# flysoaryun/LF-VIO

Hardware: AMD Instinct MI355X
Metric: sliding-window solves/sec (10 KF x N landmarks) (higher is better)
Workload: dtype f64; 1 GPU; window300; landmarks=300, observations=1419, windows_per_gpu=1, marginalization=MARGIN_OLD, parallelism=1 independent window stream(s), one per GPU, no data-path collective

## Files before the change

### lf-vio_amd/csrc/dev_types.h

```cpp
#pragma once
#include "../../include/lfvio.h"

constexpr int KC = 73;
constexpr int KP = 172;
constexpr int WLD = 80;
__host__ __device__ inline int w_row_len(int cnt) { return 6 * cnt + 9; }
constexpr int COL_B = 73;
constexpr int COL_K = 74;
constexpr int NQ = 105;
constexpr int NG = 210;
constexpr int NGP = 212;
constexpr int NPAIR = 121;
constexpr int NT = 15;
constexpr int SCHUR_LEN = NT * 256;
constexpr int PACKED = KP * (KP + 1) / 2;
constexpr int JMAX_SWEEPS = 20;
constexpr int PRE_CHUNK_LIMIT = 2 * 121;
constexpr int SUM_ITEMS_CAP = PRE_CHUNK_LIMIT * 209 + 64;
constexpr int SUM_VIS_PACKED = 73 * 74 / 2, SUM_VIS = SUM_VIS_PACKED + 73;
constexpr int HPP_CAP = 16384;
constexpr int XOFF_H = 0;
constexpr int XOFF_G = 14880;
constexpr int XOFF_S = XOFF_G + 176;
constexpr int XOFF_C = XOFF_S + 15 * 256;
// ... 167 lines not shown
  GP<int> lm_start, lm_cnt, lm_obs0, lm_perm;
  GP<int> lm_woff;
  GP<double> lam0;
  GP<double> obs[8];
  GP<int> pm_obs, pm_lm;
  GP<double> anc[8];
  GP<double> pmo[8];
  GP<unsigned char> pm_pair;
  GP<int> linb_lm0, linb_ns;
  GP<int> chunk_pair, chunk_begin, chunk_end;
  GP<double> prior_J, prior_r;
  GP<int> sum_off, sum_end_marg, sum_items;
  FrameState x[2];
  TRState tr;
  Tab tab[2];
  GP<double> lam[2];
  FrameState xE[SPEC_EXTRA];
  Tab tabE[SPEC_EXTRA];
  GP<double> lamE[SPEC_EXTRA];
  GP<double> cost_partE;
  double pose_costE[SPEC_EXTRA][16];
  double imu_sqrt[LFVIO_WINDOW_SIZE][225];
  GP<double> prior_A;
  double prior_b0[KP];
  GP<double> a, b, W, scale_l, grad_l, gn_l, diag_l, einv_l, d1, d2;
  GP<double> Wt;
  GP<double> gram_part, pairG, schur_part, schur_sum;
  GP<double> xch, gp;
  GP<double> lm_part;
  double lm_sum[LMS];
  GP<double> cost_part;
  GP<double> imu_out;
  GP<double> imu_raw;
  double prior_g[KP + 4];
  double pose_cost[16];
  GP<double> Hpp;
  GP<double> mscr;
  GP<double> eig_aux;
  double scale_p[KP], diag_p[KP], grad_p[KP], gn_p[KP], step_p[KP];
  double uc_grad[WLD], uc_gn[WLD];
  struct SpecCtl {
    int ep;
    int word;
    int fin;
    int ticket;
    int own[SPEC_OWN];
  } spec;
  struct SpecShadow {
    int hdr_ep;
    int word;
    int last_word;
    int ticket;
  } shadow;
  long long dbg[32];
  double jtrace[32];
  LfvioPrior prior_out;
};

struct PendingBlock {
  int open, passes;
  int tail_state, passes_used, iters_done, chain_err;
};
static_assert(offsetof(Slot, passes_used) - offsetof(Slot, tail_state) == offsetof(PendingBlock, passes_used) - offsetof(PendingBlock, tail_state) &&
                  offsetof(Slot, iters_done) - offsetof(Slot, tail_state) == offsetof(PendingBlock, iters_done) - offsetof(PendingBlock, tail_state) &&
                  offsetof(Slot, chain_err) - offsetof(Slot, tail_state) == offsetof(PendingBlock, chain_err) - offsetof(PendingBlock, tail_state),
              "PendingBlock mirrors Slot::tail_state .. chain_err");
```

### lf-vio_amd/csrc/kernels_marg.h

```cpp
#pragma once
#include "kernels_solve.h"

constexpr int MARG_THREADS = 768;
constexpr int MARG_MAXD = 96;
constexpr int LDN = 80;
constexpr double JACOBI_TOL = 1e-19;
constexpr size_t MARG_LDS = (size_t)19072 * sizeof(double);
constexpr int BT_GROUP = 4;

DEV void gauge_landmarks(Slot *S, int l0) {
  const int l = l0 + (int)threadIdx.x;
  double *lam = S->lam[S->tr.cur];
  if (l < S->N) lam[l] = 1.0 / (1.0 / lam[l]);
}
template <class T>
DEV void copy_rounds(T *dst, const T *src, int n, int tid, int nthr) {
  for (int k0 = tid; k0 < n; k0 += 8 * nthr) {
    T v[8];
#pragma unroll
    for (int q = 0; q < 8; q++) v[q] = src[k0 + q * nthr < n ? k0 + q * nthr : 0];
#pragma unroll
    for (int q = 0; q < 8; q++)
      if (k0 + q * nthr < n) dst[k0 + q * nthr] = v[q];
  }
// ... 561 lines not shown
#pragma unroll
  for (int i = P; i < 5; i++) {
    const double kv = K2 * vi[i];
#pragma unroll
    for (int q = P; q < 5; q++) ar[i][q] = fma(kv, vj[q], ar[i][q]);
    if (i == P) tri_finish_row<P>(tc, k + 1, ar[P], tc.r0 == ((k + 1) & 15));
  }
}
template <int QM, int NR>
DEV void bt_apply(const double *RV, const double *tau, int k, int n, int l8, double (&zz)[10]) {
  double vq[NR][10], tk[NR];
#pragma unroll
  for (int r = 0; r < NR; r++) {
    const int kr = k - r;
    const double *v = RV + kr * 76 - (kr + 1);
    tk[r] = tau[kr];
#pragma unroll
    for (int q = QM; q < 10; q++) {
      const int i = l8 + 8 * q;
      if (QM == 0) vq[r][q] = (i > kr && i < n) ? v[i] : 0.0;
      else vq[r][q] = (q > QM || i > kr) ? v[i] : 0.0;
    }
  }
#pragma unroll
  for (int r = 0; r < NR; r++) {
    double s0 = 0.0, s1 = 0.0;
#pragma unroll
    for (int q = QM; q < 10; q++) {
      if ((q - QM) & 1) s1 = fma(vq[r][q], zz[q], s1);
      else s0 = fma(vq[r][q], zz[q], s0);
    }
    const double s = sum8(s0 + s1) * tk[r];
#pragma unroll
    for (int q = QM; q < 10; q++) zz[q] = fma(-s, vq[r][q], zz[q]);
  }
}
template <int NR>
DEV void bt_dispatch(const double *RV, const double *tau, int k, int n, int l8, double (&zz)[10]) {
  switch (k >> 3) {
    case 0: bt_apply<0, NR>(RV, tau, k, n, l8, zz); break;
    case 1: bt_apply<1, NR>(RV, tau, k, n, l8, zz); break;
    case 2: bt_apply<2, NR>(RV, tau, k, n, l8, zz); break;
    case 3: bt_apply<3, NR>(RV, tau, k, n, l8, zz); break;
    case 4: bt_apply<4, NR>(RV, tau, k, n, l8, zz); break;
    case 5: bt_apply<5, NR>(RV, tau, k, n, l8, zz); break;
    case 6: bt_apply<6, NR>(RV, tau, k, n, l8, zz); break;
    case 7: bt_apply<7, NR>(RV, tau, k, n, l8, zz); break;
    case 8: bt_apply<8, NR>(RV, tau, k, n, l8, zz); break;
    default: bt_apply<9, NR>(RV, tau, k, n, l8, zz); break;
  }
}
DEV double guard_pivot(double q, double pivmin) { return copysign(fmax(fabs(q), pivmin), q); }
template <bool SPEC>
DEV bool eig_tridiag(double *A, const double *b, int n, int tid, double *RV, double *DM, double *vec, double *scr, double *nn2, double *Tglob, LfvioPrior *out, double eps, long long *dbg,
                     SpecPoll *sp_) {
  SpecPoll *const sp = SPEC ? sp_ : nullptr;
  const bool poller = SPEC && tid == MARG_THREADS - 1;
#define ESTAMP(k) do { if (tid == 0) dbg[k] = (long long)__builtin_readcyclecounter(); } while (0)
  ESTAMP(26);
  const int wave = tid >> 6, lane = tid & 63;
  double *dd = vec, *ee = vec + 96, *ee2 = vec + 192, *tau = vec + 288, *lam = vec + 384, *pp = vec + 480, *nrm = vec + 576;
  const bool tri = tid < 256;
  const int r0 = (tid >> 4) & 15, c0 = tid & 15;
  double ar[5][5];
#pragma unroll
  for (int i = 0; i < 5; i++)
#pragma unroll
    for (int q = 0; q < 5; q++) {
      const int R = r0 + 16 * i, C = c0 + 16 * q;
      ar[i][q] = (tri && R < n && C < n) ? A[max(R, C) * LDN + min(R, C)] : 0.0;
    }
  double *vb0 = lam, *vb1 = nrm;
  if (tid < 96) dd[tid] = 0.0, ee[tid] = 0.0, ee2[tid] = 0.0, tau[tid] = 0.0, vb0[tid] = 0.0, vb1[tid] = 0.0;
  for (int e = tid; e < 76 * 76; e += MARG_THREADS) RV[e] = 0.0;
  __syncthreads();
  TriCtx tc = {dd, ee, tau, vb0, vb1, pp, RV, n, r0, c0};
  if (tri) tri_finish_row<0>(tc, 0, ar[0], r0 == 0);
  __syncthreads();
  for (int k = 0; k + 2 < n; k++) {
    const int P = (k + 1) >> 4;
    double vj[5];
    if (poller) {
      if ((k & 7) == 0) spec_poll_issue(*sp);
      else if ((k & 7) == 6) spec_poll_take(*sp);
    }
#ifdef LFVIO_TRI_PROFILE
#define TSTAMP(j) do { if (tid == 0 && k == LFVIO_TRI_PROFILE) dbg[3 + j] = (long long)__builtin_readcyclecounter(); } while (0)
#else
#define TSTAMP(j) do { } while (0)
#endif
    TSTAMP(0);
    if (tri) {
      switch (P) {
        case 0: tri_matvec<0>(tc, k, ar, vj); break;
        case 1: tri_matvec<1>(tc, k, ar, vj); break;
        case 2: tri_matvec<2>(tc, k, ar, vj); break;
        case 3: tri_matvec<3>(tc, k, ar, vj); break;
        default: tri_matvec<4>(tc, k, ar, vj); break;
      }
    }
    TSTAMP(1);
    __syncthreads();
    TSTAMP(2);
    if (tri) {
      switch (P) {
        case 0: tri_update<0>(tc, k, ar, vj); break;
        case 1: tri_update<1>(tc, k, ar, vj); break;
        case 2: tri_update<2>(tc, k, ar, vj); break;
        case 3: tri_update<3>(tc, k, ar, vj); break;
        default: tri_update<4>(tc, k, ar, vj); break;
      }
    }
    TSTAMP(3);
    __syncthreads();
    TSTAMP(4);
    if (sp && (k & 7) == 6 && *sp->flag) return true;
  }
  if (tri) {
#pragma unroll
    for (int i = 0; i < 5; i++)
#pragma unroll
      for (int q = 0; q < 5; q++)
        if (r0 + 16 * i == n - 1 && c0 + 16 * q == n - 1) dd[n - 1] = ar[i][q];
  }
// ... 120 lines not shown
    __syncthreads();
    ESTAMP(17);
    if (sp && *sp->flag) return true;
    if (work) {
      const double g0 = pp[mec], g1 = pp[96 + mec];
      const int kt = g1 < g0 ? ((int *)ee2)[96 + mec] : ((int *)ee2)[mec];
      double z = 1.0, nn = 0.0;
      if (set == 0) {
        A[kt * LDN + mec] = 1.0;
        for (int i0 = n - 2; i0 >= 0; i0 -= 8) {
          double c[8], zs[8];
#pragma unroll
          for (int u = 0; u < 8; u++) {
            const int i = max(i0 - u, 0);
            c[u] = -ee[i] * fast_rcp(guard_pivot(A[i * LDN + mec], pivmin));
          }
#pragma unroll
          for (int u = 0; u < 8; u++) {
            const bool on = i0 - u < kt && i0 - u >= 0;
            z = on ? c[u] * z : 1.0;
            zs[u] = z;
            nn = on ? fma(z, z, nn) : nn;
          }
#pragma unroll
          for (int u = 0; u < 8; u++)
            if (i0 - u < kt && i0 - u >= 0) A[(i0 - u) * LDN + mec] = zs[u];
        }
      } else {
        for (int i0 = 1; i0 < n; i0 += 8) {
          double c[8], zs[8];
#pragma unroll
          for (int u = 0; u < 8; u++) {
            const int i = min(i0 + u, n - 1);
            c[u] = -ee[i - 1] * fast_rcp(guard_pivot(DM[i * LDN + mec], pivmin));
          }
#pragma unroll
          for (int u = 0; u < 8; u++) {
            const bool on = i0 + u > kt && i0 + u < n;
            z = on ? c[u] * z : 1.0;
            zs[u] = z;
            nn = on ? fma(z, z, nn) : nn;
          }
#pragma unroll
          for (int u = 0; u < 8; u++)
            if (i0 + u > kt && i0 + u < n) A[(i0 + u) * LDN + mec] = zs[u];
        }
      }
      nn2[set * 96 + mec] = nn;
    }
  }
  __syncthreads();
  ESTAMP(29);
  {
    const int m = tid >> 3, l8 = tid & 7;
    const bool live = m < n;
    const int mm = live ? m : 0;
    double zz[10];
    const double sc = fast_rsqrt(1.0 + nn2[mm] + nn2[96 + mm]);
#pragma unroll
    for (int q = 0; q < 10; q++) {
      const int i = l8 + 8 * q;
      zz[q] = i < n ? A[i * LDN + mm] * sc : 0.0;
    }
    int k = n - 3;
    for (; k >= 0 && (k & (BT_GROUP - 1)) != BT_GROUP - 1; k--) bt_dispatch<1>(RV, tau, k, n, l8, zz);
    for (; k >= 0; k -= BT_GROUP) bt_dispatch<BT_GROUP>(RV, tau, k, n, l8, zz);
    const double l = lam[mm];
    double rb = 0.0;
#pragma unroll
    for (int q = 0; q < 10; q++) {
      const int i = l8 + 8 * q;
      if (i < n) rb = fma(zz[q], b[i], rb);
    }
    rb = sum8(rb);
    if (live) {
      const bool keep = l > eps;
      const double sq = keep ? sqrt(l) : 0.0;
#pragma unroll
      for (int q = 0; q < 10; q++) {
        const int i = l8 + 8 * q;
        if (i < n) out->linearized_jacobians[m * n + i] = sq * zz[q];
      }
      if (l8 == 0) out->linearized_residuals[m] = keep ? rb / sq : 0.0;
    }
  }
  return false;
}

DEV void spec_deliver(Slot *S, Slot *S0, int my_word, bool publish) {
  const int tid = threadIdx.x, nthr = blockDim.x;
  __shared__ int give;
  if (tid == 0) {
    const int ep = spec_ep(my_word), a = spec_acc(my_word);
    long long t0 = wall_clock64();
    int g = 0;
    for (;;) {
      const int f = spec_peek(&S0->spec.fin), w = spec_peek(&S0->spec.word);
      if (spec_ep(w) != ep) break;
      const int st = spec_ep(f) == ep ? spec_fin_state(f) : FIN_OPEN;
      if (st >= FIN_MAIN) {
        g = st == FIN_SIDE && spec_fin_acc(f) == a;
        break;
      }
      if (w != my_word) break;
      if (wall_clock64() - t0 > SPEC_WAIT_TICKS) {
        if (spec_cas(&S0->spec.own[a], SPEC_SIDE, SPEC_ABANDON) == SPEC_SIDE) break;
        t0 = wall_clock64();
      }
      __builtin_amdgcn_s_sleep(8);
    }
    give = g;
  }
  __syncthreads();
  if (!give) return;
  const LfvioPrior *src = &S->prior_out;
  LfvioPrior *dst = &S0->prior_out;
  const int n = src->valid == 1 ? src->n : 0;
  copy_rounds((long long *)dst, (const long long *)src, (int)(offsetof(LfvioPrior, linearized_jacobians) / 8), tid, nthr);
  copy_rounds(dst->linearized_jacobians, src->linearized_jacobians, n * n, tid, nthr);
  copy_rounds(dst->linearized_residuals, src->linearized_residuals, n, tid, nthr);
  __syncthreads();
  if (publish) publish_prior(S0);
  char *m = (char *)S0->mail;
  if (tid == 0) {
    __threadfence_system();
    __hip_atomic_store(&S0->tail_state, (int)TAIL_DONE, __ATOMIC_RELAXED, __HIP_MEMORY_SCOPE_AGENT);
    if (m) __hip_atomic_store((int *)m + MAIL_ECHO, S->shadow.ticket, __ATOMIC_RELAXED, __HIP_MEMORY_SCOPE_SYSTEM);
  }
}

template <bool WORKER>
__global__ __launch_bounds__(MARG_THREADS) void k_marg_solve(char *base, size_t stride, int flag_bits) {
  extern __shared__ __attribute__((aligned(16))) double smem[];
  const int flag = flag_bits & 255, force_eig = (flag_bits >> 8) & 1, gated = (flag_bits >> 9) & 1;
  const int publish = (flag_bits >> 10) & 1;
  constexpr bool worker = WORKER;
  Slot *S = worker ? (Slot *)base : SLOT(base, stride);
  Slot *S0 = worker ? (Slot *)(base - stride) : S;
  __shared__ int spec_flag;
  SpecPoll sp{S0, worker ? S->shadow.word : 0, &spec_flag, 0, 0};
  if (threadIdx.x == 0) spec_flag = 0;
  const bool poller = worker && threadIdx.x == MARG_THREADS - 1;
  TRState *tr = &S->tr;
  const MargPlan *mp = &S->marg[flag];
  const int tid = threadIdx.x;
  LfvioPrior *out = &S->prior_out;
  if (gated && !tail_gate(S, tr->done)) return;
  if (worker && sp.my_word == 0) return;
  if (!mp->valid) {
    if (tid == 0) out->valid = -1;
    if (worker) {
      __syncthreads();
      spec_deliver(S, S0, sp.my_word, publish != 0);
      return;
    }
    if (gated && tid == 0) S->iters_done = tr->iteration, S->tail_state = TAIL_DONE;
    if (gated && publish) {
      __syncthreads();
      publish_prior(S);
    }
    return;
  }
  if (poller) spec_poll_issue(sp);
  STAMP(S, 10);
  const double *Sc = S->schur_sum;
  const bool sub = mp->N0 > 0 || S->sharded;
  const int m15 = mp->m15, n = mp->n, D = m15 + n;
  double *Ag = S->mscr;
  double *A = smem;
  double *bv = A + 92 * 92;
  double *Am = bv + 96;
  double *Vm = Am + 256;
  double *Ainv = Vm + 256;
  double *Tm = Ainv + 256;
  double *Ar = smem + 12544;
  double *br = Ar + 76 * LDN;
  double2 *cs = (double2 *)(br + 80);
  int *perm = (int *)(cs + 96);
  double *scr = (double *)(perm + 96);
  double *RV = smem, *vec8 = smem + 5776, *DMs = smem + 5776 + 672;
  for (int c = tid; c < KP; c += MARG_THREADS) {
    const int a = mp->col[c];
    if (a >= 0) perm[a] = c;
  }
  __syncthreads();
  {
    constexpr int GR = (92 * 92 + MARG_THREADS - 1) / MARG_THREADS;
    const double *Hp = &S->Hpp[0];
    double hv[GR], sv[GR];
#pragma unroll
    for (int k = 0; k < GR; k++) {
      const int e = tid + MARG_THREADS * k, ec = e < D * D ? e : 0;
      const int r = D ? perm[ec / max(D, 1)] : 0, c = D ? perm[ec % max(D, 1)] : 0;
      const int hi = max(r, c), lo = min(r, c);
      hv[k] = Hp[hi * (hi + 1) / 2 + lo];
      sv[k] = (sub && hi < KC) ? Sc[schur_index(lo, hi)] : 0.0;
    }
#pragma unroll
    for (int k = 0; k < GR; k++) {
      const int e = tid + MARG_THREADS * k;
      if (e < D * D) A[e] = hv[k] - sv[k];
    }
  }
  for (int a = tid; a < D; a += MARG_THREADS) {
    const int c = perm[a];
    double v = S->gp[c];
    if (sub && c < KC) v -= Sc[schur_index(c, COL_B)];
    bv[a] = v;
  }
  if (poller) spec_poll_take(sp), spec_poll_issue(sp);
  __syncthreads();
  STAMP(S, 11);
  if (worker && spec_flag) return;
  for (int e = tid; e < m15 * m15; e += MARG_THREADS) {
    const int r = e / m15, c = e % m15;
    Am[e] = 0.5 * (A[r * D + c] + A[c * D + r]);
  }
  __syncthreads();
  const double eps = 1e-8;
  __shared__ int spd_fast;
  if (tid < 64) {
    const bool fast = m15 <= 15 && !force_eig && spd_inverse_wave(Am, Ainv, m15, tid, 1e3 * eps);
    if (tid == 0) spd_fast = fast ? 1 : 0;
  }
  __syncthreads();
  int sw1 = 0;
  if (!spd_fast) {
    sw1 = jacobi_small(Am, Vm, m15, tid, MARG_THREADS, Tm, cs, scr);
    __syncthreads();
    for (int e = tid; e < m15 * m15; e += MARG_THREADS) {
      const int r = e / m15, c = e % m15;
      double s = 0;
      for (int k = 0; k < m15; k++) {
        const double ev = Am[k * m15 + k];
        if (ev > eps) s += Vm[r * m15 + k] * (1.0 / ev) * Vm[c * m15 + k];
      }
      Ainv[e] = s;
    }
    __syncthreads();
  }
  STAMP(S, 12);
  for (int e = tid; e < n * m15; e += MARG_THREADS) {
    const int r = e / m15, c = e % m15;
    double s = 0;
    for (int k = 0; k < m15; k++) s = fma(A[(m15 + r) * D + k], Ainv[k * m15 + c], s);
    Tm[e] = s;
  }
  __syncthreads();
  {
    const int nb4 = (n + 3) >> 2;
    for (int blk = tid; blk < nb4 * nb4; blk += MARG_THREADS) {
      const int r0 = 4 * (blk / nb4), c0 = 4 * (blk % nb4);
      double acc[4][4];
#pragma unroll
      for (int i = 0; i < 4; i++)
#pragma unroll
        for (int j = 0; j < 4; j++) acc[i][j] = 0.0;
      for (int k = 0; k < m15; k++) {
        double tv[4], av[4];
#pragma unroll
        for (int i = 0; i < 4; i++) tv[i] = Tm[min(r0 + i, n - 1) * m15 + k], av[i] = A[k * D + m15 + min(c0 + i, n - 1)];
#pragma unroll
        for (int i = 0; i < 4; i++)
#pragma unroll
          for (int j = 0; j < 4; j++) acc[i][j] = fma(tv[i], av[j], acc[i][j]);
      }
#pragma unroll
      for (int i = 0; i < 4; i++)
#pragma unroll
        for (int j = 0; j < 4; j++)
          if (r0 + i < n && c0 + j < n) Ar[(r0 + i) * LDN + c0 + j] = A[(m15 + r0 + i) * D + m15 + c0 + j] - acc[i][j];
    }
  }
  for (int r = tid; r < n; r += MARG_THREADS) {
    double s = 0;
    for (int k = 0; k < m15; k++) s = fma(Tm[r * m15 + k], bv[k], s);
    br[r] = bv[m15 + r] - s;
  }
  __syncthreads();
  double *Aout = Ag + 92 * 92 + 96;
  for (int e = tid; e < n * n; e += MARG_THREADS) {
    const int r = e / n, c = e % n;
    Aout[e] = Ar[max(r, c) * LDN + min(r, c)];
  }
  for (int r = tid; r < n; r += MARG_THREADS) Aout[n * n + r] = br[r];
  if (poller) spec_poll_take(sp);
  __syncthreads();
  if (worker && spec_flag) return;
  STAMP(S, 13);
  if (eig_tridiag<WORKER>(Ar, br, n, tid, RV, DMs, vec8, scr, (double *)cs, S->eig_aux, out, 1e-8, S->dbg, &sp)) return;
  if (tid == 0) S->dbg[24] = sw1;
  STAMP(S, 14);
  const FrameState *x = &S->x[tr->cur];
  if (tid < mp->nb) {
    const int kind = mp->kind[tid], frame = mp->frame[tid];
    out->blocks[tid].kind = kind;
    out->blocks[tid].frame = mp->shifted_frame[tid];
    out->block_idx[tid] = mp->idx[tid];
    const double *xb = kind == LFVIO_BLOCK_POSE ? x->pose[frame]
                       : kind == LFVIO_BLOCK_SPEEDBIAS ? x->sb[frame]
                       : kind == LFVIO_BLOCK_EX_POSE ? x->ex
                                                     : &x->td;
    const int gs = (kind == LFVIO_BLOCK_POSE || kind == LFVIO_BLOCK_EX_POSE) ? 7 : (kind == LFVIO_BLOCK_SPEEDBIAS ? 9 : 1);
    for (int k = 0; k < 9; k++) out->block_x0[tid][k] = k < gs ? xb[k] : 0.0;
  }
  STAMP(S, 15);
  if (tid == 0) {
    out->valid = 1;
    out->m = m15 + (S->sharded ? (int)(S->xch[XOFF_C + XS_N0] + 0.5) : mp->N0);
    out->n = n;
    out->num_blocks = mp->nb;
    if (gated && !worker) S->iters_done = tr->iteration, S->tail_state = TAIL_DONE;
  }
  if (worker) {
    __syncthreads();
    spec_deliver(S, S0, sp.my_word, publish != 0);
    return;
  }
  if (gated && publish) {
    __syncthreads();
    publish_prior(S);
  }
}
```

### lf-vio_amd/csrc/kernels_spec.h

```cpp
#pragma once
#include "dev_math.h"
#include "dev_types.h"

constexpr long long SPEC_WAIT_TICKS = 300000;

DEV int spec_ld(const int *p) { return __hip_atomic_load(p, __ATOMIC_ACQUIRE, __HIP_MEMORY_SCOPE_AGENT); }
DEV int spec_peek(const int *p) { return __hip_atomic_load(p, __ATOMIC_RELAXED, __HIP_MEMORY_SCOPE_AGENT); }
DEV void spec_acquire() { __builtin_amdgcn_fence(__ATOMIC_ACQUIRE, "agent"); }
DEV void spec_st(int *p, int v) { __hip_atomic_store(p, v, __ATOMIC_RELEASE, __HIP_MEMORY_SCOPE_AGENT); }
DEV int spec_cas(int *p, int expect, int v) {
  __hip_atomic_compare_exchange_strong(p, &expect, v, __ATOMIC_ACQ_REL, __ATOMIC_ACQUIRE, __HIP_MEMORY_SCOPE_AGENT);
  return expect;
}
DEV int spec_ep(int w) { return (int)((unsigned)w >> 16); }
DEV int spec_acc(int w) { return (w & 0xffff) >> 1; }
DEV int spec_fin_state(int f) { return f & 3; }
DEV int spec_fin_acc(int f) { return (f & 0xffff) >> 2; }

DEV void spec_arm(Slot *S) {
  const int ep = (S->spec.ep % 0x7fff) + 1;
  spec_st(&S->spec.word, 0);
  for (int k = 0; k < SPEC_OWN; k++) S->spec.own[k] = SPEC_FREE;
  S->spec.ep = ep;
  S->spec.ticket = S->mail ? __hip_atomic_load((const int *)S->mail + MAIL_TICKET, __ATOMIC_RELAXED, __HIP_MEMORY_SCOPE_SYSTEM) : 0;
  spec_st(&S->spec.fin, 0);
}
DEV void spec_publish(Slot *S, int num_succ, int cur) {
  if (num_succ < SPEC_OWN && S->spec.ticket != 0) spec_st(&S->spec.word, S->spec.ep << 16 | num_succ << 1 | cur);
}
DEV void spec_closing(Slot *S) {
  __hip_atomic_store(&S->spec.fin, S->spec.ep << 16 | FIN_CLOSING, __ATOMIC_SEQ_CST, __HIP_MEMORY_SCOPE_AGENT);
  __threadfence();
}
DEV bool spec_settle(Slot *S) {
  const int a = S->tr.num_succ;
  bool side = false;
  if (a < SPEC_OWN) {
    const int was = spec_cas(&S->spec.own[a], SPEC_FREE, SPEC_MAIN);
    if (was == SPEC_SIDE) side = spec_cas(&S->spec.own[a], SPEC_SIDE, SPEC_COMMIT) == SPEC_SIDE;
    if (was != SPEC_FREE && !side) spec_st(&S->spec.own[a], SPEC_MAIN);
  }
  if (side) S->tail_state = TAIL_WORKER, S->iters_done = S->tr.iteration;
  spec_st(&S->spec.fin, S->spec.ep << 16 | (a < SPEC_OWN ? a : 0) << 2 | (side ? FIN_SIDE : FIN_MAIN));
  return side;
}

DEV bool spec_stale(const Slot *S0, int my_word) {
  const int f = spec_ld(&S0->spec.fin), w = spec_ld(&S0->spec.word);
  if (spec_ep(w) != spec_ep(my_word)) return true;
  if (w != my_word) return true;
  const int st = spec_ep(f) == spec_ep(my_word) ? spec_fin_state(f) : FIN_OPEN;
  return st >= FIN_MAIN && spec_fin_acc(f) != spec_acc(my_word);
}

struct SpecPoll {
  const Slot *S0;
  int my_word;
  int *flag;
  int f, w;
};
DEV void spec_poll_issue(SpecPoll &p) {
  p.f = __hip_atomic_load(&p.S0->spec.fin, __ATOMIC_RELAXED, __HIP_MEMORY_SCOPE_AGENT);
  p.w = __hip_atomic_load(&p.S0->spec.word, __ATOMIC_RELAXED, __HIP_MEMORY_SCOPE_AGENT);
}
DEV void spec_poll_take(SpecPoll &p) {
  const int st = spec_ep(p.f) == spec_ep(p.my_word) ? spec_fin_state(p.f) : FIN_OPEN;
  if (p.w != p.my_word || (st >= FIN_MAIN && spec_fin_acc(p.f) != spec_acc(p.my_word))) *p.flag = 1;
}
```

### lf-vio_amd/csrc/lfvio_hip.hip

```cpp
#include <hip/hip_runtime.h>
#include <dlfcn.h>
typedef struct ncclComm *ncclComm_t;
#define NCCL_UNIQUE_ID_BYTES 128
typedef struct {
  char internal[NCCL_UNIQUE_ID_BYTES];
} ncclUniqueId;
typedef int ncclResult_t;
typedef int ncclDataType_t;
typedef int ncclRedOp_t;
constexpr ncclResult_t ncclSuccess = 0;
constexpr ncclRedOp_t ncclSum = 0;
constexpr ncclDataType_t ncclDouble = 8;

#include <algorithm>
#include <chrono>
#include <cmath>
#include <cstdio>
#include <cstdlib>
#include <cstring>
#include <memory>
#include <string>
#include <type_traits>
#include <vector>

// ... 131 lines not shown
struct Route {
  enum Sweep { ROLES = 0, LINW = 1, LINB = 2 } sweep;
  int count;
  Grid g;
  size_t role_wgs;
  bool split;
  int linb_gx;
  SetupLaunch setup;
  int offs;
};

struct GraphKey {
  int count = 0, lm = 0, ch = 0, sc = 0, sweep = -1, linb_gx = 0, offs = 0, setup = -1, spec = 0, passes = 0;
  bool operator==(const GraphKey &o) const {
    return count == o.count && lm == o.lm && ch == o.ch && sc == o.sc && sweep == o.sweep && linb_gx == o.linb_gx && offs == o.offs &&
           setup == o.setup && spec == o.spec && passes == o.passes;
  }
};

}

struct lfvio_ctx {
  int device = 0;
  hipStream_t stream = nullptr;
  char *d_feat = nullptr;
  size_t feat_bytes = 0;
  char *h_feat = nullptr;
  std::string err;
  int batch = 0;
  Layout L;
  char *d_base = nullptr;
  char *h_stage = nullptr;
  char *h_down = nullptr;
  size_t h_down_bytes = 0;
  std::vector<SlotHostInfo> info;
  std::vector<int> perm_build;
  hipGraphExec_t graph = nullptr;
  GraphKey graph_key;
  hipGraphExec_t chunk[2] = {}, tail[2][3] = {};
  hipGraphExec_t first[2][2][4][13] = {};
  int fixed_passes = 0;
  int recent_passes[4] = {0, 0, 0, 0}, recent_head = 0;
  int predict_passes = 4;
  double pass_seconds = 2e-4;
  GraphKey chunk_key;
  int *d_pending = nullptr;
  PendingBlock *h_pending = nullptr;
  CallState call;
  char *h_mail = nullptr, *d_mail = nullptr;
  hipStream_t fstream = nullptr;
  static constexpr int WORKERS = 2;
  hipStream_t sstream[WORKERS] = {};
  bool shadow = false;
  bool marg_ahead = true;
  hipGraphExec_t side[WORKERS][2][2] = {};
  long long stat_ahead_calls = 0, stat_ahead_hits = 0;
  hipEvent_t stage_event = nullptr;
  bool stage_busy = false;
  double up_us[4] = {0, 0, 0, 0};
  std::unique_ptr<LfvioPrior> held;
  int mail_seq = 0;
  std::unique_ptr<LfvioPrior> chain_struct;
  char *d_relo = nullptr, *h_relo = nullptr;
  size_t relo_dev_cap = 0, relo_stage_cap = 0;
  int relo_done_word = 0;
  bool relo_force = false;
  bool debug_break_chain = false;
  bool use_graph = true;
  int stat_chunks = 0;
  int last_passes = 0;
  int last_iters = 0;
  bool fixed_spec = false;
  int spec_count = 3;
  int *d_lwt = nullptr;
  int *d_asm = nullptr;
  bool shard_group = false;
  int shard_kmax0 = -1;
  int lm_half = 1;
  int linw_mode = 1;
  double init_radius = 1e4;
  double fn_tol = 1e-6;
  bool force_eig = false;
  bool shard_active = false;
  int shard_begin = 0, shard_end = 0, shard_state = 0;
  std::vector<int> sh_start, sh_off;
  static constexpr int FLAG_RING = 4;
  int *h_flags = nullptr;
  hipEvent_t flag_event[FLAG_RING] = {};
  long long flag_head = 0, flag_tail = 0;
};

namespace {

void destroy_graph(lfvio_ctx *c, bool keep_side = false) {
  if (c->stream && c->call.graphs_dropped()) (void)hipStreamSynchronize(c->stream);
  if (c->graph) {
    (void)hipGraphExecDestroy(c->graph);
    c->graph = nullptr;
  }
  if (!keep_side) {
    for (auto &st : c->sstream)
      if (st) (void)hipStreamSynchronize(st);
    for (auto &wk : c->side)
      for (auto &row : wk)
        for (auto &t : row)
          if (t) (void)hipGraphExecDestroy(t), t = nullptr;
// ... 1628 lines not shown
    for (int ci = 0; ci < 6 * lcn[dl] + 7; ci++)
      W[(size_t)perm[dl] * KC + (ci < 6 * lcn[dl] ? 6 * lst[dl] + ci : 66 + (ci - 6 * lcn[dl]))] = Wv[(size_t)woff[dl] + ci];
  }
  *cost = tr.x_cost;
  return LFVIO_OK;
}

int lfvio_debug_schur_repeat(lfvio_ctx *c, const LfvioWindow *in, double mu, double *max_abs_diff) {
  if (!c || !in || !max_abs_diff) return LFVIO_ERR_ARG;
  (void)hipSetDevice(c->device);
  int rc = reserve(c, 1, in->num_landmarks, in->num_observations);
  if (rc) return rc;
  if ((rc = upload_window(c, 0, in))) return rc;
  const Route r = route_for(c, 1, MODE_SOLVE);
  char *d = c->d_base;
  const size_t o_tr = offsetof(Slot, tr);
  auto poke_int = [&](size_t off, int v) { return hipMemcpy(d + o_tr + off, &v, sizeof v, hipMemcpyHostToDevice); };
  auto run = [&](int do_lin, std::vector<double> &out) -> int {
    HIPCHK(c, hipMemcpy(d + o_tr + offsetof(TRState, mu), &mu, sizeof mu, hipMemcpyHostToDevice));
    HIPCHK(c, poke_int(offsetof(TRState, do_lin), do_lin));
    HIPCHK(c, poke_int(offsetof(TRState, do_schur), 1));
    launch_sweep(c, r, MODE_SOLVE, true);
    HIPCHK(c, hipGetLastError());
    HIPCHK(c, hipStreamSynchronize(c->stream));
    out.resize(SCHUR_LEN);
    HIPCHK(c, hipMemcpy(out.data(), d + c->L.xch + sizeof(double) * XOFF_S, sizeof(double) * SCHUR_LEN, hipMemcpyDeviceToHost));
    return LFVIO_OK;
  };
  launch_setup(c, r, MODE_SOLVE);
  HIPCHK(c, hipStreamSynchronize(c->stream));
  std::vector<double> first, repeat, full;
  const double mu1 = mu;
  mu = 1e-8;
  if ((rc = run(1, first))) return rc;
  launch_solve(c, 1, r.sweep == Route::LINW);
  HIPCHK(c, hipStreamSynchronize(c->stream));
  mu = mu1;
  if ((rc = run(0, repeat))) return rc;
  if ((rc = run(1, full))) return rc;
  double m = 0, ref = 0;
  for (int i = 0; i < SCHUR_LEN; i++) m = std::max(m, std::fabs(repeat[i] - full[i])), ref = std::max(ref, std::fabs(full[i] - first[i]));
  *max_abs_diff = m;
  return ref > 0 ? LFVIO_OK : LFVIO_ERR_ARG;
}

int lfvio_debug_marg_system(lfvio_ctx *c, int n, double *A, double *b) {
  if (!c || !c->d_base) return LFVIO_ERR_ARG;
  (void)hipSetDevice(c->device);
  if (int rc = join_inflight(c)) return rc;
  if (n < 0 || n > 76) return LFVIO_ERR_ARG;
  if (n == 0) return LFVIO_OK;
  char *d = c->d_base + c->L.mscr;
  if (c->shadow) {
    const size_t head = offsetof(LfvioPrior, linearized_jacobians), bytes = head + sizeof(double) * n * n;
    std::vector<char> p0(bytes), pw(bytes);
    HIPCHK(c, hipMemcpy(p0.data(), c->d_base + offsetof(Slot, prior_out), bytes, hipMemcpyDeviceToHost));
    const LfvioPrior *h0 = (const LfvioPrior *)p0.data();
    for (int wk = 0; wk < lfvio_ctx::WORKERS && h0->valid == 1 && h0->n == n; wk++) {
      char *ds = c->d_base + (size_t)(c->batch + wk) * c->L.total;
      HIPCHK(c, hipMemcpy(pw.data(), ds + offsetof(Slot, prior_out), bytes, hipMemcpyDeviceToHost));
      const LfvioPrior *hw = (const LfvioPrior *)pw.data();
      if (hw->valid == 1 && hw->n == n && std::memcmp(p0.data() + head, pw.data() + head, bytes - head) == 0) {
        d = ds + c->L.mscr;
        break;
      }
    }
  }
  HIPCHK(c, hipMemcpy(A, d + sizeof(double) * (92 * 92 + 96), sizeof(double) * n * n, hipMemcpyDeviceToHost));
  HIPCHK(c, hipMemcpy(b, d + sizeof(double) * (92 * 92 + 96 + n * n), sizeof(double) * n, hipMemcpyDeviceToHost));
  return LFVIO_OK;
}

int lfvio_debug_read_clocks(lfvio_ctx *c, long long *out32) {
  if (!c || !c->d_base) return LFVIO_ERR_ARG;
  if (int rc = join_inflight(c)) return rc;
  HIPCHK(c, hipMemcpy(out32, c->d_base + offsetof(Slot, dbg), sizeof(long long) * 32, hipMemcpyDeviceToHost));
  HIPCHK(c, hipMemcpy(out32 + 32, c->d_base + offsetof(Slot, jtrace), sizeof(double) * 32, hipMemcpyDeviceToHost));
  return LFVIO_OK;
}

int lfvio_debug_time_kernel(lfvio_ctx *c, int which, int count, int reps, double *avg_ms) {
  if (!c || !c->d_base || count <= 0 || count > c->batch || reps <= 0) return LFVIO_ERR_ARG;
  (void)hipSetDevice(c->device);
  if (int rc = join_inflight(c)) return rc;
  const Route r = route_for(c, count, MODE_SOLVE);
  const Grid &g = r.g;
  const size_t st = c->L.total;
  const bool lw = r.sweep == Route::LINW, lb = r.sweep == Route::LINB;
  const bool offs = (r.offs & 2) != 0;
  if ((which == 11 || which == 12) && !lw) {
    c->err = "the resident windows are not linearized by k_linw";
    return LFVIO_ERR_ARG;
  }
  if (which >= 15 && which <= 17 && !lb) {
    c->err = "the resident window is not linearized by k_linb";
    return LFVIO_ERR_ARG;
  }
  hipEvent_t e0, e1;
  HIPCHK(c, hipEventCreate(&e0));
  if (hipError_t e = hipEventCreate(&e1); e != hipSuccess) {
    (void)hipEventDestroy(e0);
    HIPCHK(c, e);
  }
  launch_setup(c, r, MODE_SOLVE);
  Route full = r;
  if (lb && !(which >= 15 && which <= 17)) full.sweep = Route::ROLES;
  launch_sweep(c, full, MODE_SOLVE, offs);
  if (which == 14) launch_solve(c, count, lw);
  if (which == 17) launch_solve(c, count, false);

  HIPCHK(c, hipEventRecord(e0, c->stream));
  for (int rep = 0; rep < reps; rep++) {
    switch (which) {
      case 0: launch_lin(c, r, MODE_SOLVE, offs); break;
      case 2: launch_sum(c, r, MODE_SOLVE); break;
      case 8: case 9: case 10: case 18: {
        const int gram_wgs = (g.ch + 3) / 4;
        const int gx = which == 8 ? g.lw : which == 9 ? gram_wgs : which == 18 ? LFVIO_WINDOW_SIZE : LFVIO_WINDOW_SIZE + 1;
        hipLaunchKernelGGL((k_lin<LIN_ROLE_ALL, false>), dim3(gx, count), dim3(LIN_THREADS), 0, c->stream, c->d_base, st, MODE_SOLVE, which == 8 ? g.lw : 0,
                           which == 9 ? gram_wgs : 0);
      } break;
      case 4: case 5: case 6: case 7: {
        const SetupLaunch sl = setup_launch(c, count, g.lm, false);
        const int wgs = (sl.bits & 4) ? 3 : SETUP_WGS, gx = which == 4 ? 1 : which == 5 ? 2 : which == 6 ? wgs : sl.gx;
        hipLaunchKernelGGL(k_setup, dim3(gx, count), dim3(256), 0, c->stream, c->d_base, st, MODE_SOLVE, sl.bits);
      } break;
      case 11: case 12: launch_sweep(c, r, MODE_SOLVE, offs); break;
      case 13: launch_solve(c, count, lw); break;
      case 14: hipLaunchKernelGGL(k_stepw, dim3(1, count), dim3(STEPW_LAUNCH_THREADS), 0, c->stream, c->d_base, st); break;
      case 15: hipLaunchKernelGGL(k_linb<false>, dim3(r.linb_gx, count), dim3(LW_THREADS), LW_LDS_BYTES, c->stream, c->d_base, st, linw_args(c)); break;
// ... 31 lines not shown
  HIPCHK(c, hipGetLastError());
  HIPCHK(c, hipStreamSynchronize(c->stream));
  const char *d = c->d_base + (size_t)slot * st;
  const int N = c->info[slot].N;
  auto get = [&](double *dst, size_t off, size_t n) { return !dst || !n ? hipSuccess : hipMemcpy(dst, d + off, n * 8, hipMemcpyDeviceToHost); };
  HIPCHK(c, get(gp, c->L.xch + (size_t)XOFF_G * 8, KP));
  HIPCHK(c, get(schur, c->L.xch + (size_t)XOFF_S * 8, SCHUR_LEN));
  HIPCHK(c, get(lm_sum, offsetof(Slot, lm_sum), 5));
  HIPCHK(c, get(a, c->L.a, N));
  HIPCHK(c, get(b, c->L.b, N));
  HIPCHK(c, get(gn_p, offsetof(Slot, gn_p), KP));
  HIPCHK(c, get(q, offsetof(Slot, tr) + offsetof(TRState, q), Q_COUNT));
  HIPCHK(c, get(x_cost, offsetof(Slot, tr) + offsetof(TRState, x_cost), 1));
  return r.sweep;
}

int lfvio_debug_configure(lfvio_ctx *c, const char *key, double value) {
  if (!c || !key) return LFVIO_ERR_ARG;
  const std::string k = key;
  const int iv = (int)value;
  if (k == "env") {
    const char *e = getenv("LFVIO_DEBUG");
    if (!e) return LFVIO_OK;
    std::string all = e;
    for (size_t p = 0; p < all.size();) {
      const size_t q = std::min(all.find(',', p), all.size()), eq = all.find('=', p);
      if (eq != std::string::npos && eq < q) {
        const int rc = lfvio_debug_configure(c, all.substr(p, eq - p).c_str(), atof(all.substr(eq + 1, q - eq - 1).c_str()));
        if (rc) return rc;
      }
      p = q + 1;
    }
    return LFVIO_OK;
  }
  const bool structural = k == "graph" || k == "linw" || k == "force_eig";
  if (structural) {
    if (int rc = join_inflight(c)) return rc;
  }
  if (k == "graph") c->use_graph = iv != 0;
  else if (k == "first_passes") {
    if (iv < 0) return LFVIO_ERR_ARG;
    c->fixed_passes = iv;
  } else if (k == "spec_count") c->fixed_spec = iv > 0, c->spec_count = iv > 0 ? std::max(1, std::min(1 + SPEC_EXTRA, iv)) : 3;
  else if (k == "function_tolerance") {
    if (!(value >= 0.0)) return LFVIO_ERR_ARG;
    c->fn_tol = value;
  } else if (k == "initial_radius") c->init_radius = value > 0.0 ? value : 1e4;
  else if (k == "linw") {
    if (iv < 0 || iv > 2) return LFVIO_ERR_ARG;
    c->linw_mode = iv;
  } else if (k == "lm_half") c->lm_half = iv != 0;
  else if (k == "force_eig") c->force_eig = iv != 0;
  else if (k == "marg_ahead") c->marg_ahead = iv != 0;
  else if (k == "break_next_chain") c->debug_break_chain = iv != 0;
  else if (k == "relo_route") c->relo_force = iv != 0;
  else {
    c->err = "lfvio_debug_configure: unknown key '" + k + "'";
    return LFVIO_ERR_ARG;
  }
  if (structural) destroy_graph(c);
  return LFVIO_OK;
}

int lfvio_debug_query(lfvio_ctx *c, const char *key, double *out, int n) {
  if (!c || !key || !out || n <= 0) return LFVIO_ERR_ARG;
  const std::string k = key;
  auto put = [&](std::initializer_list<double> v) {
    int i = 0;
    for (double x : v)
      if (i < n) out[i++] = x;
    return LFVIO_OK;
  };
  if (k == "last_call") return put({(double)c->last_passes, (double)c->last_iters, (double)c->stat_chunks, (double)c->spec_count});
  if (k == "marg_ahead") return put({(double)c->stat_ahead_calls, (double)c->stat_ahead_hits});
  if (k == "upload_times") return put({c->up_us[0], c->up_us[1], c->up_us[2], c->up_us[3]});
  if (k == "sweep_kernel") {
    const int r = sweep_kernel_of(c, (int)out[0]);
    if (r < 0) return r;
    return put({(double)r});
  }
  c->err = "lfvio_debug_query: unknown key '" + k + "'";
  return LFVIO_ERR_ARG;
}

#include "relo.inc"
#include "feat.inc"

#include "twoview.inc"

#include "vialign.inc"

#include "pnp.inc"
#include "shard.inc"
#include "group.inc"

}
```

### lf-vio_amd/lfvio/engine.py

```python
import ctypes as C

import numpy as np

from . import abi

_dp = C.POINTER(C.c_double)


def _p(a):
    return a.ctypes.data_as(_dp)


class Engine:
    def __init__(self, device=0, lib_path=None):
        self.lib = abi.load_hip_library(lib_path)
        self.lib.lfvio_debug_linearize.argtypes = [C.c_void_p, C.POINTER(abi.WindowC), _dp, _dp, _dp, _dp, _dp, _dp]
        self.lib.lfvio_debug_marg_system.argtypes = [C.c_void_p, C.c_int, _dp, _dp]
        self.lib.lfvio_debug_configure.argtypes = [C.c_void_p, C.c_char_p, C.c_double]
        self.lib.lfvio_debug_query.argtypes = [C.c_void_p, C.c_char_p, _dp, C.c_int]
        self.lib.lfvio_debug_time_kernel.argtypes = [C.c_void_p, C.c_int, C.c_int, C.c_int, _dp]
        self.ctx = self.lib.lfvio_create(device)
        if not self.ctx:
            raise RuntimeError("lfvio_create failed: no usable HIP device (there is no CPU fallback)")

    def close(self):
        if self.ctx:
            self.lib.lfvio_destroy(self.ctx)
            self.ctx = None

    def __del__(self):
        try:
            self.close()
        except Exception:
            pass

    def _check(self, rc, what):
        if rc != 0:
            raise RuntimeError(f"{what} failed rc={rc}: {self.lib.lfvio_last_error(self.ctx).decode()}")

    def configure(self, key, value=1.0):
        self._check(self.lib.lfvio_debug_configure(self.ctx, key.encode(), float(value)), f"lfvio_debug_configure({key})")

    def query(self, key, n, first=0.0):
        out = np.zeros(max(n, 1))
        out[0] = first
        self._check(self.lib.lfvio_debug_query(self.ctx, key.encode(), _p(out), n), f"lfvio_debug_query({key})")
        return out

    def set_graph(self, on):
        self.configure("graph", int(on))

    def marg_ahead(self, on=-1):
        if on >= 0:
            self.configure("marg_ahead", int(on))
        q = self.query("marg_ahead", 2)
        return int(q[0]), int(q[1])

    def break_next_chain(self):
        self.configure("break_next_chain", 1)

    def set_lm_half(self, on):
        self.configure("lm_half", int(on))

    def set_initial_radius(self, r):
        self.configure("initial_radius", float(r))

    def set_linw(self, mode):
        self.configure("linw", int(mode))

    def resident_pass(self, count, slot, n_landmarks):
        out = dict(gp=np.zeros(abi.KP), schur=np.zeros(15 * 256), lm_sum=np.zeros(5), a=np.zeros(max(n_landmarks, 1)),
                   b=np.zeros(max(n_landmarks, 1)), gn_p=np.zeros(abi.KP), q=np.zeros(16), x_cost=np.zeros(1))
        dp = C.POINTER(C.c_double)
        self.lib.lfvio_debug_resident_pass.argtypes = [C.c_void_p, C.c_int, C.c_int] + [dp] * 8
        rc = self.lib.lfvio_debug_resident_pass(self.ctx, count, slot, *[_p(out[k]) for k in ("gp", "schur", "lm_sum", "a", "b", "gn_p", "q", "x_cost")])
        if rc < 0:
            self._check(rc, "resident_pass")
        out["a"], out["b"], out["linw"] = out["a"][:n_landmarks], out["b"][:n_landmarks], rc
        return out

    def set_function_tolerance(self, tol):
        self.configure("function_tolerance", float(tol))

    def last_chunks(self):
        return int(self.query("last_call", 4)[2])

    def last_passes(self):
        return int(self.query("last_call", 4)[0])

    def force_eig(self, on):
        self.configure("force_eig", int(on))

    def solve(self, win):
        sol = abi.Solution(win.N)
        self._check(self.lib.lfvio_solve(self.ctx, C.byref(win.c()), C.byref(sol.c)), "lfvio_solve")
        return sol

    def solve_relo(self, win, frame, relo_pose, landmark=(), match_point=()):
        relo = abi.Relo(frame, relo_pose, landmark, match_point)
        rc_ = relo.c()
        sol = abi.Solution(win.N)
        out = np.zeros(abi.SIZE_POSE)
        self._check(self.lib.lfvio_solve_relo(self.ctx, C.byref(win.c()), C.byref(rc_), C.byref(sol.c), _p(out)), "lfvio_solve_relo")
        return sol, out

    def solve_relo_rc(self, win, relo, sol, out, num_matches=None, null_arrays=False):
        rc_ = relo.c(num_matches=num_matches, null_arrays=null_arrays)
        return int(self.lib.lfvio_solve_relo(self.ctx, C.byref(win.c()), C.byref(rc_), C.byref(sol.c), _p(out)))
# ... 371 lines not shown
```

Baseline: 2414 solves/s.

## Write committed speculative marginal prior directly into main slot, skip copy

When a speculative worker learns during polling that its result was committed, it writes the linearized Jacobians and residuals straight into the main slot's prior output and skips the later copy rounds in spec_deliver. The dense A/b export is folded into eig_tridiag using the idle threads above 256. The prior block metadata writes are moved earlier so they overlap the Schur section. The spec poll also moves ahead of the export, so abandoned workers exit sooner. Adds delivery counters, a deliv_from offset that replaces the host memcmp search in the debug path, and a worker-clocks debug option, at the cost of more complex commit-state handling.

```diff
diff --git a/lf-vio_amd/csrc/dev_types.h b/lf-vio_amd/csrc/dev_types.h
--- a/lf-vio_amd/csrc/dev_types.h
+++ b/lf-vio_amd/csrc/dev_types.h
@@ -243,6 +243,8 @@
     int last_word;
     int ticket;
   } shadow;
+  int deliv_direct, deliv_copied;
+  long long deliv_from;
   long long dbg[32];
   double jtrace[32];
   LfvioPrior prior_out;
diff --git a/lf-vio_amd/csrc/kernels_marg.h b/lf-vio_amd/csrc/kernels_marg.h
--- a/lf-vio_amd/csrc/kernels_marg.h
+++ b/lf-vio_amd/csrc/kernels_marg.h
@@ -637,7 +637,7 @@
 }
 DEV double guard_pivot(double q, double pivmin) { return copysign(fmax(fabs(q), pivmin), q); }
 template <bool SPEC>
-DEV bool eig_tridiag(double *A, const double *b, int n, int tid, double *RV, double *DM, double *vec, double *scr, double *nn2, double *Tglob, LfvioPrior *out, double eps, long long *dbg,
+DEV bool eig_tridiag(double *A, const double *b, int n, int tid, double *RV, double *DM, double *vec, double *scr, double *nn2, double *Tglob, double *Aout, LfvioPrior *out, LfvioPrior *out_direct, double eps, long long *dbg,
                      SpecPoll *sp_) {
   SpecPoll *const sp = SPEC ? sp_ : nullptr;
   const bool poller = SPEC && tid == MARG_THREADS - 1;
@@ -655,6 +655,17 @@
       const int R = r0 + 16 * i, C = c0 + 16 * q;
       ar[i][q] = (tri && R < n && C < n) ? A[max(R, C) * LDN + min(R, C)] : 0.0;
     }
+  if (!tri) {
+    const int nt = MARG_THREADS - 256, t = tid - 256, nd = max(n, 1);
+    const int dr = nt / nd, dc = nt - dr * nd;
+    int r = t / nd, c = t - r * nd;
+    for (int e = t; e < n * n; e += nt) {
+      Aout[e] = A[max(r, c) * LDN + min(r, c)];
+      r += dr, c += dc;
+      if (c >= n) c -= n, r++;
+    }
+    if (t < n) Aout[n * n + t] = b[t];
+  }
   double *vb0 = lam, *vb1 = nrm;
   if (tid < 96) dd[tid] = 0.0, ee[tid] = 0.0, ee2[tid] = 0.0, tau[tid] = 0.0, vb0[tid] = 0.0, vb1[tid] = 0.0;
   for (int e = tid; e < 76 * 76; e += MARG_THREADS) RV[e] = 0.0;
@@ -881,6 +892,7 @@
   __syncthreads();
   ESTAMP(29);
   {
+    LfvioPrior *const o = (SPEC && *sp->committed) ? out_direct : out;
     const int m = tid >> 3, l8 = tid & 7;
     const bool live = m < n;
     const int mm = live ? m : 0;
@@ -908,18 +920,20 @@
 #pragma unroll
       for (int q = 0; q < 10; q++) {
         const int i = l8 + 8 * q;
-        if (i < n) out->linearized_jacobians[m * n + i] = sq * zz[q];
-      }
-      if (l8 == 0) out->linearized_residuals[m] = keep ? rb / sq : 0.0;
+        if (i < n) o->linearized_jacobians[m * n + i] = sq * zz[q];
+      }
+      if (l8 == 0) o->linearized_residuals[m] = keep ? rb / sq : 0.0;
     }
   }
   return false;
 }
 
-DEV void spec_deliver(Slot *S, Slot *S0, int my_word, bool publish) {
+DEV void spec_deliver(Slot *S, Slot *S0, int my_word, bool publish, bool direct) {
   const int tid = threadIdx.x, nthr = blockDim.x;
   __shared__ int give;
-  if (tid == 0) {
+  if (direct) {
+    if (tid == 0) give = 1;
+  } else if (tid == 0) {
     const int ep = spec_ep(my_word), a = spec_acc(my_word);
     long long t0 = wall_clock64();
     int g = 0;
@@ -946,12 +960,16 @@
   LfvioPrior *dst = &S0->prior_out;
   const int n = src->valid == 1 ? src->n : 0;
   copy_rounds((long long *)dst, (const long long *)src, (int)(offsetof(LfvioPrior, linearized_jacobians) / 8), tid, nthr);
-  copy_rounds(dst->linearized_jacobians, src->linearized_jacobians, n * n, tid, nthr);
-  copy_rounds(dst->linearized_residuals, src->linearized_residuals, n, tid, nthr);
+  if (!direct) {
+    copy_rounds(dst->linearized_jacobians, src->linearized_jacobians, n * n, tid, nthr);
+    copy_rounds(dst->linearized_residuals, src->linearized_residuals, n, tid, nthr);
+  }
   __syncthreads();
   if (publish) publish_prior(S0);
   char *m = (char *)S0->mail;
   if (tid == 0) {
+    (void)__hip_atomic_fetch_add(direct ? &S0->deliv_direct : &S0->deliv_copied, 1, __ATOMIC_RELAXED, __HIP_MEMORY_SCOPE_AGENT);
+    S0->deliv_from = (long long)((char *)S - (char *)S0);
     __threadfence_system();
     __hip_atomic_store(&S0->tail_state, (int)TAIL_DONE, __ATOMIC_RELAXED, __HIP_MEMORY_SCOPE_AGENT);
     if (m) __hip_atomic_store((int *)m + MAIL_ECHO, S->shadow.ticket, __ATOMIC_RELAXED, __HIP_MEMORY_SCOPE_SYSTEM);
@@ -966,9 +984,9 @@
   constexpr bool worker = WORKER;
   Slot *S = worker ? (Slot *)base : SLOT(base, stride);
   Slot *S0 = worker ? (Slot *)(base - stride) : S;
-  __shared__ int spec_flag;
-  SpecPoll sp{S0, worker ? S->shadow.word : 0, &spec_flag, 0, 0};
-  if (threadIdx.x == 0) spec_flag = 0;
+  __shared__ int spec_flag, spec_committed;
+  SpecPoll sp{S0, worker ? S->shadow.word : 0, &spec_flag, 0, 0, &spec_committed};
+  if (threadIdx.x == 0) spec_flag = 0, spec_committed = 0;
   const bool poller = worker && threadIdx.x == MARG_THREADS - 1;
   TRState *tr = &S->tr;
   const MargPlan *mp = &S->marg[flag];
@@ -980,7 +998,7 @@
     if (tid == 0) out->valid = -1;
     if (worker) {
       __syncthreads();
-      spec_deliver(S, S0, sp.my_word, publish != 0);
+      spec_deliver(S, S0, sp.my_word, publish != 0, false);
       return;
     }
     if (gated && tid == 0) S->iters_done = tr->iteration, S->tail_state = TAIL_DONE;
@@ -1012,6 +1030,10 @@
     const int a = mp->col[c];
     if (a >= 0) perm[a] = c;
   }
+  const int pb = tid - 8 * 64;
+  const bool pblk = pb >= 0 && pb < mp->nb;
+  int pb_kind = 0, pb_frame = 0, pb_shifted = 0, pb_idx = 0;
+  if (pblk) pb_kind = mp->kind[pb], pb_frame = mp->frame[pb], pb_shifted = mp->shifted_frame[pb], pb_idx = mp->idx[pb];
   __syncthreads();
   {
     constexpr int GR = (92 * 92 + MARG_THREADS - 1) / MARG_THREADS;
@@ -1025,10 +1047,28 @@
       hv[k] = Hp[hi * (hi + 1) / 2 + lo];
       sv[k] = (sub && hi < KC) ? Sc[schur_index(lo, hi)] : 0.0;
     }
+    double pb_x[9];
+    if (pblk) {
+      const FrameState *x = &S->x[tr->cur];
+      const double *xb = pb_kind == LFVIO_BLOCK_POSE ? x->pose[pb_frame]
+                         : pb_kind == LFVIO_BLOCK_SPEEDBIAS ? x->sb[pb_frame]
+                         : pb_kind == LFVIO_BLOCK_EX_POSE ? x->ex
+                                                          : &x->td;
+      const int gs = (pb_kind == LFVIO_BLOCK_POSE || pb_kind == LFVIO_BLOCK_EX_POSE) ? 7 : (pb_kind == LFVIO_BLOCK_SPEEDBIAS ? 9 : 1);
+#pragma unroll
+      for (int k = 0; k < 9; k++) pb_x[k] = k < gs ? xb[k] : 0.0;
+    }
 #pragma unroll
     for (int k = 0; k < GR; k++) {
       const int e = tid + MARG_THREADS * k;
       if (e < D * D) A[e] = hv[k] - sv[k];
+    }
+    if (pblk) {
+      out->blocks[pb].kind = pb_kind;
+      out->blocks[pb].frame = pb_shifted;
+      out->block_idx[pb] = pb_idx;
+#pragma unroll
+      for (int k = 0; k < 9; k++) out->block_x0[pb][k] = pb_x[k];
     }
   }
   for (int a = tid; a < D; a += MARG_THREADS) {
@@ -1106,44 +1146,26 @@
     for (int k = 0; k < m15; k++) s = fma(Tm[r * m15 + k], bv[k], s);
     br[r] = bv[m15 + r] - s;
   }
-  __syncthreads();
+  if (poller) spec_poll_take(sp);
+  __syncthreads();
+  if (worker && spec_flag) return;
   double *Aout = Ag + 92 * 92 + 96;
-  for (int e = tid; e < n * n; e += MARG_THREADS) {
-    const int r = e / n, c = e % n;
-    Aout[e] = Ar[max(r, c) * LDN + min(r, c)];
-  }
-  for (int r = tid; r < n; r += MARG_THREADS) Aout[n * n + r] = br[r];
-  if (poller) spec_poll_take(sp);
-  __syncthreads();
-  if (worker && spec_flag) return;
   STAMP(S, 13);
-  if (eig_tridiag<WORKER>(Ar, br, n, tid, RV, DMs, vec8, scr, (double *)cs, S->eig_aux, out, 1e-8, S->dbg, &sp)) return;
+  if (eig_tridiag<WORKER>(Ar, br, n, tid, RV, DMs, vec8, scr, (double *)cs, S->eig_aux, Aout, out, &S0->prior_out, 1e-8, S->dbg, &sp)) return;
   if (tid == 0) S->dbg[24] = sw1;
   STAMP(S, 14);
-  const FrameState *x = &S->x[tr->cur];
-  if (tid < mp->nb) {
-    const int kind = mp->kind[tid], frame = mp->frame[tid];
-    out->blocks[tid].kind = kind;
-    out->blocks[tid].frame = mp->shifted_frame[tid];
-    out->block_idx[tid] = mp->idx[tid];
-    const double *xb = kind == LFVIO_BLOCK_POSE ? x->pose[frame]
-                       : kind == LFVIO_BLOCK_SPEEDBIAS ? x->sb[frame]
-                       : kind == LFVIO_BLOCK_EX_POSE ? x->ex
-                                                     : &x->td;
-    const int gs = (kind == LFVIO_BLOCK_POSE || kind == LFVIO_BLOCK_EX_POSE) ? 7 : (kind == LFVIO_BLOCK_SPEEDBIAS ? 9 : 1);
-    for (int k = 0; k < 9; k++) out->block_x0[tid][k] = k < gs ? xb[k] : 0.0;
-  }
   STAMP(S, 15);
   if (tid == 0) {
     out->valid = 1;
     out->m = m15 + (S->sharded ? (int)(S->xch[XOFF_C + XS_N0] + 0.5) : mp->N0);
     out->n = n;
     out->num_blocks = mp->nb;
+    if (!worker) S->deliv_from = 0;
     if (gated && !worker) S->iters_done = tr->iteration, S->tail_state = TAIL_DONE;
   }
   if (worker) {
     __syncthreads();
-    spec_deliver(S, S0, sp.my_word, publish != 0);
+    spec_deliver(S, S0, sp.my_word, publish != 0, spec_committed != 0);
     return;
   }
   if (gated && publish) {
diff --git a/lf-vio_amd/csrc/kernels_spec.h b/lf-vio_amd/csrc/kernels_spec.h
--- a/lf-vio_amd/csrc/kernels_spec.h
+++ b/lf-vio_amd/csrc/kernels_spec.h
@@ -58,6 +58,7 @@
   int my_word;
   int *flag;
   int f, w;
+  int *committed;
 };
 DEV void spec_poll_issue(SpecPoll &p) {
   p.f = __hip_atomic_load(&p.S0->spec.fin, __ATOMIC_RELAXED, __HIP_MEMORY_SCOPE_AGENT);
@@ -66,4 +67,8 @@
 DEV void spec_poll_take(SpecPoll &p) {
   const int st = spec_ep(p.f) == spec_ep(p.my_word) ? spec_fin_state(p.f) : FIN_OPEN;
   if (p.w != p.my_word || (st >= FIN_MAIN && spec_fin_acc(p.f) != spec_acc(p.my_word))) *p.flag = 1;
+  if (st == FIN_SIDE && spec_fin_acc(p.f) == spec_acc(p.my_word)) {
+    spec_acquire();
+    *p.committed = 1;
+  }
 }
diff --git a/lf-vio_amd/csrc/lfvio_hip.hip b/lf-vio_amd/csrc/lfvio_hip.hip
--- a/lf-vio_amd/csrc/lfvio_hip.hip
+++ b/lf-vio_amd/csrc/lfvio_hip.hip
@@ -207,6 +207,7 @@
   static constexpr int WORKERS = 2;
   hipStream_t sstream[WORKERS] = {};
   bool shadow = false;
+  bool clocks_of_worker = false;
   bool marg_ahead = true;
   hipGraphExec_t side[WORKERS][2][2] = {};
   long long stat_ahead_calls = 0, stat_ahead_hits = 0;
@@ -1941,19 +1942,10 @@
   if (n == 0) return LFVIO_OK;
   char *d = c->d_base + c->L.mscr;
   if (c->shadow) {
-    const size_t head = offsetof(LfvioPrior, linearized_jacobians), bytes = head + sizeof(double) * n * n;
-    std::vector<char> p0(bytes), pw(bytes);
-    HIPCHK(c, hipMemcpy(p0.data(), c->d_base + offsetof(Slot, prior_out), bytes, hipMemcpyDeviceToHost));
-    const LfvioPrior *h0 = (const LfvioPrior *)p0.data();
-    for (int wk = 0; wk < lfvio_ctx::WORKERS && h0->valid == 1 && h0->n == n; wk++) {
-      char *ds = c->d_base + (size_t)(c->batch + wk) * c->L.total;
-      HIPCHK(c, hipMemcpy(pw.data(), ds + offsetof(Slot, prior_out), bytes, hipMemcpyDeviceToHost));
-      const LfvioPrior *hw = (const LfvioPrior *)pw.data();
-      if (hw->valid == 1 && hw->n == n && std::memcmp(p0.data() + head, pw.data() + head, bytes - head) == 0) {
-        d = ds + c->L.mscr;
-        break;
-      }
-    }
+    long long from = 0;
+    HIPCHK(c, hipMemcpy(&from, c->d_base + offsetof(Slot, deliv_from), sizeof(from), hipMemcpyDeviceToHost));
+    if (from < 0 || (size_t)from > (size_t)(c->batch + lfvio_ctx::WORKERS - 1) * c->L.total || (size_t)from % c->L.total) return LFVIO_ERR_ARG;
+    d += from;
   }
   HIPCHK(c, hipMemcpy(A, d + sizeof(double) * (92 * 92 + 96), sizeof(double) * n * n, hipMemcpyDeviceToHost));
   HIPCHK(c, hipMemcpy(b, d + sizeof(double) * (92 * 92 + 96 + n * n), sizeof(double) * n, hipMemcpyDeviceToHost));
@@ -1963,8 +1955,15 @@
 int lfvio_debug_read_clocks(lfvio_ctx *c, long long *out32) {
   if (!c || !c->d_base) return LFVIO_ERR_ARG;
   if (int rc = join_inflight(c)) return rc;
-  HIPCHK(c, hipMemcpy(out32, c->d_base + offsetof(Slot, dbg), sizeof(long long) * 32, hipMemcpyDeviceToHost));
-  HIPCHK(c, hipMemcpy(out32 + 32, c->d_base + offsetof(Slot, jtrace), sizeof(double) * 32, hipMemcpyDeviceToHost));
+  const char *d = c->d_base;
+  if (c->clocks_of_worker && c->shadow) {
+    long long from = 0;
+    HIPCHK(c, hipMemcpy(&from, c->d_base + offsetof(Slot, deliv_from), sizeof(from), hipMemcpyDeviceToHost));
+    if (from < 0 || (size_t)from > (size_t)(c->batch + lfvio_ctx::WORKERS - 1) * c->L.total || (size_t)from % c->L.total) return LFVIO_ERR_ARG;
+    d += from;
+  }
+  HIPCHK(c, hipMemcpy(out32, d + offsetof(Slot, dbg), sizeof(long long) * 32, hipMemcpyDeviceToHost));
+  HIPCHK(c, hipMemcpy(out32 + 32, d + offsetof(Slot, jtrace), sizeof(double) * 32, hipMemcpyDeviceToHost));
   return LFVIO_OK;
 }
 
@@ -2102,6 +2101,7 @@
   } else if (k == "lm_half") c->lm_half = iv != 0;
   else if (k == "force_eig") c->force_eig = iv != 0;
   else if (k == "marg_ahead") c->marg_ahead = iv != 0;
+  else if (k == "clocks_of_worker") c->clocks_of_worker = iv != 0;
   else if (k == "break_next_chain") c->debug_break_chain = iv != 0;
   else if (k == "relo_route") c->relo_force = iv != 0;
   else {
@@ -2123,6 +2123,14 @@
   };
   if (k == "last_call") return put({(double)c->last_passes, (double)c->last_iters, (double)c->stat_chunks, (double)c->spec_count});
   if (k == "marg_ahead") return put({(double)c->stat_ahead_calls, (double)c->stat_ahead_hits});
+  if (k == "marg_direct") {
+    int cnt[2] = {0, 0};
+    if (c->d_base) {
+      if (int rc = join_inflight(c)) return rc;
+      HIPCHK(c, hipMemcpy(cnt, c->d_base + offsetof(Slot, deliv_direct), sizeof(cnt), hipMemcpyDeviceToHost));
+    }
+    return put({(double)cnt[0], (double)cnt[1]});
+  }
   if (k == "upload_times") return put({c->up_us[0], c->up_us[1], c->up_us[2], c->up_us[3]});
   if (k == "sweep_kernel") {
     const int r = sweep_kernel_of(c, (int)out[0]);
diff --git a/lf-vio_amd/lfvio/engine.py b/lf-vio_amd/lfvio/engine.py
--- a/lf-vio_amd/lfvio/engine.py
+++ b/lf-vio_amd/lfvio/engine.py
@@ -54,6 +54,10 @@
         if on >= 0:
             self.configure("marg_ahead", int(on))
         q = self.query("marg_ahead", 2)
+        return int(q[0]), int(q[1])
+
+    def marg_direct(self):
+        q = self.query("marg_direct", 2)
         return int(q[0]), int(q[1])
 
     def break_next_chain(self):
```

New measurement: 2421 solves/s, median of 6. About the same (+0.3%).
